# chintha/U-VIP-SLAM

Hardware: AMD Instinct MI355X
Metric: frames/sec ORB extract+match, 640x512 @1000 kp (higher is better)
Workload: dtype u8; 1 GPU; BASELINE.json configs[2]: 1xMI355X per rank, batch=256 synthetic 640x512 mono frames (+1 halo frame: the neighbouring rank's first), 1000 feats, 8 levels, fastTh 20, FullDetect extract + all-pairs 256-bit Hamming knn-2 of consecutive frames, HBM-resident I/O; batch_per_gpu=256, pipeline_depth=2, input_batches_in_rotation=4, fast_mode=adaptive

## Files before the change

u-vip-slam_amd/__init__.py:

```python
import ctypes
import os

import numpy as np

_HERE = os.path.dirname(os.path.abspath(__file__))
LIB_PATH = os.path.join(_HERE, "libuvo.so")

KEYPOINT_DTYPE = np.dtype([("x", "<f4"), ("y", "<f4"), ("size", "<f4"), ("angle", "<f4"), ("response", "<f4"), ("octave", "<i4"),
                           ("class_id", "<i4")])
assert KEYPOINT_DTYPE.itemsize == 28

UVO_OK, UVO_E_BADARG, UVO_E_NODEVICE, UVO_E_HIP, UVO_E_CAPACITY, UVO_E_UNSUPPORTED, UVO_E_NOMEM = 0, -1, -2, -3, -4, -5, -6
UVO_TUNE_OCT_WIDE_MAX = 1
UVO_TUNE_FAST_MODE = 2
UVO_FAST_MODE_ADAPTIVE, UVO_FAST_MODE_TWO_PASS, UVO_FAST_MODE_SINGLE_PASS = 0, 1, 2
UVO_TUNE_BLUR_ROUNDING, UVO_BLUR_ROUNDING_SCALAR, UVO_BLUR_ROUNDING_SSE2 = 9, 0, 1
UVO_TUNE_LEVEL0_INPLACE = 11
UVO_TUNE_FUSE_BLUR_TREE = 10
UVO_TUNE_PYR_RING = 12
UVO_TUNE_PYR_FORM, UVO_PYR_FORM_AUTO, UVO_PYR_FORM_LEVELS, UVO_PYR_FORM_TILES = 13, 0, 1, 2
UVO_TUNE_PYR_TILE_GROUP = 14
UVO_TUNE_FEW_FRAMES = 16
UVO_TUNE_ZERO_COPY_OUT, UVO_TUNE_SPIN_WAIT = 17, 18

ABI_SYMBOLS = [
    "uvo_extractor_create", "uvo_extractor_destroy", "uvo_extractor_levels", "uvo_extractor_max_keypoints", "uvo_extractor_scale_factor", "uvo_extractor_tables",
    "uvo_extract", "uvo_extract_tracked", "uvo_extract_batch", "uvo_extract_batch_device", "uvo_host_alloc", "uvo_host_free", "uvo_host_register", "uvo_host_unregister", "uvo_host_bind_near_device", "uvo_host_bind_to_cpulist_file", "uvo_shard_plan_make", "uvo_sharder_create", "uvo_sharder_destroy", "uvo_sharder_max_keypoints", "uvo_sharder_run", "uvo_sharder_submit", "uvo_sharder_wait", "uvo_extract_batch_submit", "uvo_extract_batch_wait", "uvo_extractor_synchronize", "uvo_extractor_set_pipeline", "uvo_extractor_tune", "uvo_extractor_fast_state", "uvo_extractor_level_dims",
    "uvo_grider_fast", "uvo_clahe", "uvo_clahe_batch_device", "uvo_extractor_read_plane", "uvo_extractor_read_candidates", "uvo_extractor_profile", "uvo_extractor_profile_only", "uvo_extractor_kernel_times",
    "uvo_matcher_create", "uvo_matcher_destroy", "uvo_matcher_synchronize", "uvo_hamming_knn2", "uvo_hamming_knn2_batch_device",
    "uvo_hamming_matrix", "uvo_distinctive_descriptors", "uvo_search_by_projection", "uvo_match_windows", "uvo_match_groups",
    "uvo_search_by_projection_kf", "uvo_search_by_bow", "uvo_search_for_triangulation", "uvo_search_for_triangulation_batch", "uvo_search_for_triangulation_next", "uvo_triangulate_matches", "uvo_create_new_map_points", "uvo_fuse", "uvo_fuse_batch", "uvo_project_points", "uvo_search_points_in_frustum", "uvo_sim3_decompose", "uvo_sim3_relative", "uvo_project_sim3", "uvo_search_by_projection_sim3", "uvo_search_by_sim3", "uvo_haloc_hash", "uvo_klt_create", "uvo_klt_destroy", "uvo_klt_build_pyramid", "uvo_klt_build_pyramid_from_extractor", "uvo_klt_read_level", "uvo_klt_track", "uvo_undistort_points", "uvo_klt_track_undistorted", "uvo_klt_find_fundamental", "uvo_klt_track_filtered", "uvo_klt_fm_hypotheses", "uvo_klt_solve_pnp_ransac", "uvo_klt_pnp_hypotheses", "uvo_vocabulary_create", "uvo_vocabulary_destroy", "uvo_bow_transform", "uvo_matcher_wait_extractor", "uvo_extractor_wait_matcher", "uvo_matcher_attach_extractor", "uvo_matcher_profile",
    "uvo_glibc_srand", "uvo_glibc_rand_next", "uvo_pnpsolver_set_create", "uvo_pnpsolver_set_destroy", "uvo_pnpsolver_set_clear", "uvo_pnpsolver_add",
    "uvo_pnpsolver_query", "uvo_pnpsolver_iterate", "uvo_pnpsolver_hypotheses",
    "uvo_sim3solver_set_create", "uvo_sim3solver_set_destroy", "uvo_sim3solver_set_clear", "uvo_sim3solver_add", "uvo_sim3solver_set_ransac_parameters",
    "uvo_sim3solver_query", "uvo_sim3solver_iterate", "uvo_sim3solver_find", "uvo_sim3solver_hypotheses",
    "uvo_initializer_create", "uvo_initializer_destroy", "uvo_initializer_set_reference", "uvo_initializer_initialize", "uvo_initializer_hypotheses",
    "uvo_matcher_kernel_times", "uvo_last_error", "uvo_device_info",
]


class MatchRule(ctypes.Structure):
    _fields_ = [("rule", ctypes.c_int32), ("max_dist", ctypes.c_int32), ("nn_ratio", ctypes.c_float), ("exclusive", ctypes.c_int32),
                ("check_orientation", ctypes.c_int32)]


class FeatureVectorC(ctypes.Structure):
    _fields_ = [("node", ctypes.c_void_p), ("start", ctypes.c_void_p), ("feat", ctypes.c_void_p), ("n_nodes", ctypes.c_int32)]


class Epipolar(ctypes.Structure):
    _fields_ = [("f12", ctypes.c_float * 9), ("q_x", ctypes.c_void_p), ("q_y", ctypes.c_void_p), ("t_x", ctypes.c_void_p), ("t_y", ctypes.c_void_p),
                ("sigma2", ctypes.c_void_p), ("nlevels", ctypes.c_int32)]


class CameraPose(ctypes.Structure):
    _fields_ = [("rcw", ctypes.c_float * 9), ("tcw", ctypes.c_float * 3), ("ow", ctypes.c_float * 3), ("fx", ctypes.c_float), ("fy", ctypes.c_float),
                ("cx", ctypes.c_float), ("cy", ctypes.c_float), ("min_x", ctypes.c_float), ("max_x", ctypes.c_float), ("min_y", ctypes.c_float),
                ("max_y", ctypes.c_float)]

    @classmethod
    def make(cls, Rcw, tcw, Ow, fx, fy, cx, cy, bounds):
        c = cls()
        c.rcw[:] = [float(x) for x in np.asarray(Rcw, np.float32).reshape(9)]
        c.tcw[:] = [float(x) for x in np.asarray(tcw, np.float32).reshape(3)]
        c.ow[:] = [float(x) for x in np.asarray(Ow, np.float32).reshape(3)]
        c.fx, c.fy, c.cx, c.cy = float(fx), float(fy), float(cx), float(cy)
        c.min_x, c.min_y, c.max_x, c.max_y = [float(b) for b in bounds]
        return c

    def as_array(self):
        return np.frombuffer(bytes(self), np.float32).copy()


# ... 1543 lines not shown
```

u-vip-slam_amd/csrc/common.hpp:

```cpp
#pragma once
#include "strip_plan.hpp"
#include "pyr_tiles.hpp"
#include <hip/hip_runtime.h>
#include <stdint.h>

#include "../../include/uvo/uvo.h"

namespace uvo {

constexpr int kMaxLevels = 16;
constexpr int kPad = 16;
constexpr int kPyrPitchAlign = 64;
constexpr int kMinBorder = 13;
constexpr int kMaxOctN = 2000;

struct LevelGeom {
  int w, h;
  int pw, ph, pitch;
  int64_t plane_off;
  int bw, bh;
  int nCols, nRows, wCell, hCell;
  int cell_base;
  int n_cells;
  int quota;
  int cand_cap;
  int64_t cand_off;
  int sel_cap;
  int sel_off;
  int nIni;
  float hX;
  float scale;
  float patch_size;
  int xtab_off;
  int ytab_off;
  int oct_tab_off;
  int pad_;
};

struct Level0View {
  const uint8_t* vbase;
  int64_t frame_stride;
  int pitch;
  int pad;
};

struct CellDesc {
  int16_t level;
  int16_t x0, y0;
  int16_t rw, rh;
  int16_t ox, oy;
  int16_t pad;
};

struct Geom {
  int width, height, nlevels;
  int total_cells;
  int64_t pyr_block;
  int64_t cand_block;
  int sel_block;
  int flist_cap;
  LevelGeom lv[kMaxLevels];
};


struct FinalSlot {
  float x, y;
  int32_t level;
  int32_t aux;
};

struct LaneScratch {
  uint8_t *pyr = nullptr, *blur = nullptr;
  uint32_t *cand_xy = nullptr, *cand_sc = nullptr, *cand_lo = nullptr, *pstate = nullptr, *sel_xy = nullptr, *sel_sc = nullptr;
  int32_t *cand_count = nullptr, *sel_count = nullptr, *n_final = nullptr, *cor_n = nullptr, *cursor = nullptr;
  uint32_t* cor = nullptr;
  uint8_t* cell_hi = nullptr;
  int32_t *tpass = nullptr, *fstat = nullptr, *fcount = nullptr;
  uint2* cell_list = nullptr;
  FinalSlot* flist = nullptr;
};

const char* hip_err_set(hipError_t e, const char* what);
#ifdef __HIPCC__
__device__ __forceinline__ int wave_in_block() { return __builtin_amdgcn_readfirstlane((int)(threadIdx.x >> 6)); }
#endif

int fail(int code, const char* msg);
int dev_malloc(void** p, size_t bytes);

#define UVO_HIP_CHECK(expr)                                   \
  do {                                                        \
    hipError_t _e = (expr);                                   \
    if (_e != hipSuccess) {                                   \
      uvo::hip_err_set(_e, #expr);                            \
      return UVO_E_HIP;                                       \
    }                                                         \
  } while (0)

#define RC(call)                   \
  do {                             \
    const int _rc = (call);        \
    if (_rc != UVO_OK) return _rc; \
  } while (0)

void launch_pad_level0(hipStream_t s, const uint8_t* d_img, int w, int h, int64_t stride, int64_t frame_stride, uint8_t* d_pyr,
                       int64_t pyr_block, const LevelGeom& g0, int batch);
void launch_resize_level(hipStream_t s, uint8_t* d_pyr, int64_t pyr_block, const LevelGeom& src, const LevelGeom& dst, const ResizeCol* d_ctab,
                         const ResizeRow* d_rtab, int fast_ok, int batch, Level0View l0, int ring);
constexpr int kPyrTilesMaxLds = 160 * 1024;
int prepare_pyr_tiles(uint32_t* max_lds);
int launch_pyr_tiles(hipStream_t s, uint8_t* d_pyr, int64_t pyr_block, const PyrTileLevel* d_plan, const Geom& g, const ResizeCol* d_ctab, const ResizeRow* d_rtab,
                     Level0View l0, int first, int last, int ntiles, uint32_t lds_bytes, int threads, int rows, int batch);
void launch_gauss7(hipStream_t s, const uint8_t* d_pyr, uint8_t* d_blur, int64_t pyr_block, const LevelGeom* d_lv, const Geom& g, int4 taps,
                   int batch, int sse2_rounding, Level0View l0);
void launch_fast_score(hipStream_t s, const LaneScratch& d, const Geom& g, int fast_th, int batch, Level0View l0);
void launch_fast_cells(hipStream_t s, const LaneScratch& d, const Geom& g, const CellDesc* d_cells, const int32_t* d_flag_cell, int batch, Level0View l0);
void launch_grider(hipStream_t s, const uint8_t* d_img, int w, int h, int64_t stride, int num_features, int grid_x, int grid_y, int threshold,
                   int nms, uint8_t* d_score, uint32_t* d_lists, int32_t* d_counts, uvo_keypoint* d_out, int cap, int32_t* d_n_out);
int fast_rows_per_seg(int batch);
int fast_items_per_frame(const Geom& g, int rows_per_seg);
int fast_flags_per_frame(const Geom& g);
struct OctLaunchState {
  int wide_max_problems = 0;
};
bool octree_gauss_applies(const OctLaunchState& st, const Geom& g, int batch);
void launch_octree_gauss(hipStream_t s, const LevelGeom* d_lv, const Geom& g, const LaneScratch& d, int4 taps, int sse2_rounding, int batch, Level0View l0,
                         const uint16_t* d_oct_tab);
int prepare_octree(const Geom& g);
void octree_fill_path_tables(const Geom& g, uint16_t* dst);
int launch_octree(hipStream_t s, OctLaunchState& st, const LevelGeom* d_lv, const Geom& g, const LaneScratch& d, int batch, const uint16_t* d_oct_tab);
struct FastAdapt {
  const int32_t* fcount;
  int32_t* tpass;
  int32_t* last;
  int adapt, fast_th;
};
void launch_assemble(hipStream_t s, const LevelGeom* d_lv, const Geom& g, FastAdapt fa, const LaneScratch& d, const int32_t* d_n_in, int in_cap,
                     int32_t* d_grid, int grid_rows, int grid_cols, int min_px_dist, int full_detect, const int32_t* d_nfn, int batch);
void launch_occupancy_grid(hipStream_t s, const uvo_keypoint* d_in_kp, const int32_t* d_n_in, int in_cap, int min_px_dist, int grid_rows, int grid_cols,
                           int32_t* d_grid, int batch);
void launch_knn2(hipStream_t s, int pairs, int max_q, const uint8_t* d_q, const int32_t* d_nq, int nq_fixed, int q_stride, const uint8_t* d_t,
                 const int32_t* d_nt, int nt_fixed, int t_stride, const uint8_t* d_mask, int out_stride, int32_t* d_idx0, uint16_t* d_d0,
                 int32_t* d_idx1, uint16_t* d_d1);
void launch_medoid(hipStream_t s, const uint8_t* d_desc, const int32_t* d_offsets, int npoints, int32_t* d_idx, int32_t* d_med);
void launch_matrix(hipStream_t s, const uint8_t* d_q, int nq, const uint8_t* d_t, int nt, uint16_t* d_dist);
void launch_grid_build(hipStream_t s, const uvo_keypoint* d_kp, const uint8_t* d_desc, int n, int min_x, int min_y, int max_x, int max_y,
                       int32_t* d_cell_start, int32_t* d_cell_items, int32_t* d_cell_of_kp);
void launch_sbp(hipStream_t s, const uvo_keypoint* d_kp, int n, const uint8_t* d_desc, int min_x, int min_y, int max_x, int max_y,
                int32_t* d_assigned, int nmp, const float* d_px, const float* d_py, const int32_t* d_level, const float* d_vc,
                const uint8_t* d_inview, const uint8_t* d_mpdesc, const float* d_scale, float th, float nnratio, int32_t* d_cell_start,
                int32_t* d_cell_items, int32_t* d_cell_of_kp, int32_t* d_cand_cnt, int32_t* d_cand_start, uint32_t* d_cand, int32_t* d_owner,
                int32_t* d_owner_next, int32_t* d_choice, int32_t* d_n_matches, int stage, int64_t cand_cap);
void launch_project(hipStream_t s, int mode, const uvo_camera_pose& cam, int n, const float* d_xyz, const float* d_normal, const float* d_min,
                    const float* d_max, const float* d_max_raw, const uint8_t* d_usable, const float* d_sf, int nlevels, float log_sf, float cos_limit,
                    uint8_t* d_valid, float* d_u, float* d_v, int32_t* d_level, float* d_cos);
void launch_project_sim3(hipStream_t s, const float* r_own, const float* t_own, const float* s_r, const float* t, const uvo_camera_pose& cam, int n,
                         const float* d_xyz, const float* d_min, const float* d_max, const uint8_t* d_usable, const float* d_sf, int nlevels,
                         uint8_t* d_valid, float* d_u, float* d_v, int32_t* d_level);
void launch_haloc(hipStream_t s, const float* d_proj, int num_proj, int proj_stride, const uint8_t* d_desc, int n, float* d_hash);
void launch_win_count(hipStream_t s, const uvo_keypoint* d_kp, const uint8_t* d_desc, int n, int min_x, int min_y, int max_x, int max_y, int nq,
                      const float* d_qx, const float* d_qy, const float* d_qr, const int32_t* d_qmin, const int32_t* d_qmax,
// ... 37 lines not shown
```

u-vip-slam_amd/csrc/extractor.cpp:

```cpp
#include <algorithm>
#include <chrono>
#include <cstdio>
#include <cstring>
#include <mutex>
#include <vector>

#include "extractor_priv.hpp"
#include "fast_geom.hpp"

namespace uvo {

static thread_local char g_err[512] = "";
const char* hip_err_set(hipError_t e, const char* what) {
  snprintf(g_err, sizeof(g_err), "HIP error %d (%s) in %s", (int)e, hipGetErrorString(e), what);
  return g_err;
}
int fail(int code, const char* msg) {
  snprintf(g_err, sizeof(g_err), "%s", msg);
  return code;
}

int dev_malloc(void** p, size_t bytes) {
  const hipError_t e = hipMalloc(p, bytes);
  if (e != hipSuccess) {
// ... 143 lines not shown

struct ProfScope : Profiler::Scope {
  ProfScope(uvo_extractor* h, const char* name) : Profiler::Scope(&h->prof, name, h->lane[h->cur].stream) {}
};

int run_batch_device(uvo_extractor* h, int li, const Batch& b) {
  if (!h || !b.imgs || !b.out_kp || !b.out_desc || !b.n_out) return fail(UVO_E_BADARG, "null pointer");
  const int batch = b.n, width = b.width, height = b.height, cap = b.cap, full_detect = b.full_detect;
  const ptrdiff_t stride = b.stride, frame_stride = b.frame_stride;
  const uint8_t* const d_imgs = b.imgs;
  if (batch < 1 || batch > h->cfg.max_batch) return fail(UVO_E_BADARG, "batch outside 1..max_batch");
  if (width < 1 || height < 1 || stride < width || cap < 1) return fail(UVO_E_BADARG, "bad image size / stride / cap");
  if (!full_detect && (!b.grid || !b.nfn || b.min_px_dist < 1 || b.grid_rows < 1 || b.grid_cols < 1))
    return fail(UVO_E_BADARG, "top-up mode needs grid2d, num_feats_needed and min_px_dist >= 1");
  if (!full_detect && (b.grid_rows <= (height - 1) / b.min_px_dist || b.grid_cols <= (width - 1) / b.min_px_dist))
    return fail(UVO_E_BADARG, "grid2d smaller than ceil(image / min_px_dist)");
  UVO_HIP_CHECK(hipSetDevice(h->device));
  int rc = set_geometry(h, width, height);
  if (rc) return rc;
  if ((rc = prepare_octree(h->geom)) != UVO_OK) return rc;
  h->cur = li;
  Lane& L = h->lane[li];
  hipStream_t s = L.stream;
  {
    std::lock_guard<std::mutex> lk(h->followers_mu);
    for (uvo_matcher* m : h->followers) uvo_matcher_follow_internal(m, s);
  }
  h->last_batch = batch;
  const Geom& g = h->geom;
  hipEvent_t& done = L.done[L.n_enqueued & 1];
  if (done) UVO_HIP_CHECK(hipEventSynchronize(done));
  else UVO_HIP_CHECK(hipEventCreateWithFlags(&done, hipEventDisableTiming));
  const bool have_in = b.in_kp && b.n_in;
  const bool inplace = h->level0_inplace && width % 4 == 0 && stride % 4 == 0 && frame_stride % 4 == 0 &&
                       (uintptr_t)d_imgs % 4 == 0 && !have_in && width >= 64 && height >= 64 &&
                       stride <= (1 << 20) && (int64_t)(height + 2 * kPad) * stride < (int64_t)1 << 31;
  Level0View l0{nullptr, 0, 0, 0};
  if (inplace) l0 = Level0View{d_imgs - (int64_t)kPad * stride - kPad, (int64_t)frame_stride, (int)stride, 0};
  L.l0_src = inplace ? d_imgs : nullptr, L.l0_stride = stride, L.l0_frame_stride = frame_stride;
  L.ring_used = h->pyr_ring;
  const Level0View no_l0{nullptr, 0, 0, 0};
  {
    if (!inplace) {
      ProfScope p(h, "k_pad_level0");
      launch_pad_level0(s, d_imgs, width, height, stride, frame_stride, L.d.pyr, g.pyr_block, g.lv[0], batch);
    }
    const bool tiles = h->pyr_ring == 4 && !h->tile_groups.empty() && (h->pyr_form == UVO_PYR_FORM_TILES || (h->pyr_form == UVO_PYR_FORM_AUTO && batch <= kTilePyramidFrames));
    if (tiles) {
      for (const TileGroup& G : h->tile_groups) {
        ProfScope p(h, "k_pyr_tiles");
        launch_pyr_tiles(s, L.d.pyr, g.pyr_block, G.d_plan, g, h->d_ctab, h->d_rtab, l0, G.first, G.last, G.tx * G.ty, G.lds, G.threads, G.rows, batch);
      }
    } else {
      for (int l = 1; l < g.nlevels; ++l) {
        ProfScope p(h, "k_resize_level");
        launch_resize_level(s, L.d.pyr, g.pyr_block, g.lv[l - 1], g.lv[l], h->d_ctab + g.lv[l].xtab_off, h->d_rtab + g.lv[l].ytab_off, h->resize_fast[l],
                            batch, l == 1 ? l0 : no_l0, h->pyr_ring);
      }
    }
  }
  const bool fused_tree = h->fuse_blur_tree && octree_gauss_applies(h->oct, g, batch);
  const bool few = batch <= kFewFrames && h->few_frames_shape;
  const int4 gtaps = make_int4(h->gtaps[0], h->gtaps[1], h->gtaps[2], h->gtaps[3]);
  {
    ProfScope p(h, "k_fast_score");
    launch_fast_score(s, L.d, g, h->cfg.fast_th, batch, l0);
  }
  if (h->cfg.fast_th > 7 && h->fast_mode != UVO_FAST_MODE_SINGLE_PASS) {
    ProfScope p(h, "k_fast_cells");
    launch_fast_cells(s, L.d, g, h->d_cells, h->d_cell_flag, batch, l0);
  }
  if (fused_tree) {
    ProfScope p(h, "k_octree_gauss");
    launch_octree_gauss(s, h->d_lv, g, L.d, gtaps, h->blur_rounding, batch, l0, h->d_oct_tab);
  } else {
    {
      ProfScope p(h, "k_gauss7");
      launch_gauss7(s, L.d.pyr, L.d.blur, g.pyr_block, h->d_lv, g, gtaps, batch, h->blur_rounding, l0);
    }
    {
      ProfScope p(h, "k_octree");
      rc = launch_octree(s, h->oct, h->d_lv, g, L.d, batch, h->d_oct_tab);
      if (rc) return rc;
    }
  }
  const bool direct = few && full_detect && !have_in;
  const FastAdapt fa{L.d.fcount, L.d.tpass, L.d.fstat, h->fast_mode == UVO_FAST_MODE_ADAPTIVE ? 1 : 0, h->cfg.fast_th};
  if (!direct) {
    ProfScope p(h, "k_assemble");
    launch_assemble(s, h->d_lv, g, fa, L.d, b.n_in, h->cfg.max_input_keypoints, b.grid, b.grid_rows, b.grid_cols, b.min_px_dist, full_detect, b.nfn, batch);
  }
  {
    ProfScope p(h, "k_describe");
    if (direct) launch_describe_direct(s, h->d_lv, g, L.d, fa, h->d_pattern, h->d_patch, b.out_kp, b.out_desc, cap, b.n_out, batch, l0);
    else launch_describe(s, h->d_lv, g, L.d, b.in_kp, h->cfg.max_input_keypoints, h->d_pattern, h->d_patch, b.out_kp, b.out_desc, cap, b.n_out, batch, l0);
  }
  UVO_HIP_CHECK(hipGetLastError());
  UVO_HIP_CHECK(hipEventRecord(done, s));
  L.n_enqueued++;
  return UVO_OK;
}

static int fill_lane(uvo_extractor* h, int li) {
  Lane& L = h->lane[li];
  LaneScratch& d = L.d;
  const size_t B = (size_t)h->cfg.max_batch;
  const hipError_t e = hipStreamCreateWithFlags(&L.stream, hipStreamNonBlocking);
  if (e != hipSuccess) {
    L.stream = nullptr;
    hip_err_set(e, "hipStreamCreate");
// ... 208 lines not shown
                           double clip_limit, int tiles_x, int tiles_y, uint8_t* d_dst, ptrdiff_t dst_stride, ptrdiff_t dst_frame_stride) {
  if (!h || !d_imgs || !d_dst) return fail(UVO_E_BADARG, "null pointer");
  if (stride < width || dst_stride < width) return fail(UVO_E_BADARG, "stride smaller than the row");
  UVO_HIP_CHECK(hipSetDevice(h->device));
  int tw, th, clip;
  float scale;
  int rc = clahe_setup(h, batch, width, height, clip_limit, tiles_x, tiles_y, &tw, &th, &clip, &scale);
  if (rc) return rc;
  Lane& L = h->lane[next_lane(h)];
  {
    Profiler::Scope ps(&h->prof, "k_clahe", L.stream);
    launch_clahe(L.stream, d_imgs, width, height, stride, frame_stride, batch, tiles_x, tiles_y, tw, th, clip, scale, h->d_clahe_lut, d_dst, dst_stride,
                 dst_frame_stride);
  }
  UVO_HIP_CHECK(hipGetLastError());
  return UVO_OK;
}

int uvo_extractor_max_keypoints(const uvo_extractor* h) {
  if (!h) return fail(UVO_E_BADARG, "null handle");
  return h->cap_flist;
}

int uvo_extractor_synchronize(uvo_extractor* h) {
  if (!h) return fail(UVO_E_BADARG, "null handle");
  UVO_HIP_CHECK(hipSetDevice(h->device));
  if (h->spin_wait && h->last_batch > 0 && h->last_batch <= 16) {
    for (int i = 0; i < kMaxLanes; ++i)
      if (h->lane[i].stream) UVO_HIP_CHECK(wait_stream(h->lane[i].stream, true));
    return UVO_OK;
  }
  return sync_all_lanes(h);
}

int uvo_extractor_tune(uvo_extractor* h, int knob, int value) {
  if (!h) return fail(UVO_E_BADARG, "null handle");
  switch (knob) {
    case UVO_TUNE_OCT_WIDE_MAX:
      if (value < 0) return fail(UVO_E_BADARG, "knob value must be >= 0");
      h->oct.wide_max_problems = value;
      return UVO_OK;
    case UVO_TUNE_FAST_MODE: {
      if (value != UVO_FAST_MODE_ADAPTIVE && value != UVO_FAST_MODE_TWO_PASS && value != UVO_FAST_MODE_SINGLE_PASS)
        return fail(UVO_E_BADARG, "UVO_TUNE_FAST_MODE takes UVO_FAST_MODE_ADAPTIVE / _TWO_PASS / _SINGLE_PASS");
      UVO_HIP_CHECK(hipSetDevice(h->device));
      int rc = sync_all_lanes(h);
      if (rc) return rc;
      h->fast_mode = value;
      for (int i = 0; i < kMaxLanes; ++i)
        if (h->lane[i].stream && (rc = set_lane_fast_mode(h, i)) != UVO_OK) return rc;
      return UVO_OK;
    }
    case UVO_TUNE_PYR_FORM:
      if (value < UVO_PYR_FORM_AUTO || value > UVO_PYR_FORM_TILES) return fail(UVO_E_BADARG, "UVO_TUNE_PYR_FORM takes UVO_PYR_FORM_AUTO / _LEVELS / _TILES");
      h->pyr_form = value;
      return UVO_OK;
    case UVO_TUNE_PYR_TILE_GROUP: {
      const int first = (value >> 16) & 0xff, tx = (value >> 8) & 0xff, ty = value & 0xff;
      if (value != 0 && (first < 1 || first >= kMaxLevels || tx < 1 || ty < 1 || (first > 1 && (h->tile_spec.empty() || first <= (int)((h->tile_spec.back() >> 16) & 0xff)))))
        return fail(UVO_E_BADARG, "UVO_TUNE_PYR_TILE_GROUP takes first << 16 | tx << 8 | ty with ascending first levels starting at 1, or 0");
      UVO_HIP_CHECK(hipSetDevice(h->device));
      int rc = sync_all_lanes(h);
      if (rc) return rc;
      if (value == 0 || first == 1) h->tile_spec.clear();
      if (value != 0) h->tile_spec.push_back((uint32_t)value);
      return h->have_geom ? build_tile_groups(h, h->geom) : UVO_OK;
    }
    case UVO_TUNE_PYR_RING:
      if (value != 0 && value != 4 && value != 8 && value != 12) return fail(UVO_E_BADARG, "UVO_TUNE_PYR_RING takes 0, 4, 8 or 12");
      h->pyr_ring = value;
      return UVO_OK;
    case UVO_TUNE_LEVEL0_INPLACE:
      h->level0_inplace = value != 0;
      return UVO_OK;
    case UVO_TUNE_ZERO_COPY_OUT:
      h->zero_copy_out = value != 0;
      return UVO_OK;
    case UVO_TUNE_SPIN_WAIT:
      h->spin_wait = value != 0;
      return UVO_OK;
    case UVO_TUNE_FEW_FRAMES:
      h->few_frames_shape = value != 0;
      return UVO_OK;
    case UVO_TUNE_FUSE_BLUR_TREE:
      h->fuse_blur_tree = value != 0;
      return UVO_OK;
    case UVO_TUNE_BLUR_ROUNDING:
      if (value != UVO_BLUR_ROUNDING_SCALAR && value != UVO_BLUR_ROUNDING_SSE2) return fail(UVO_E_BADARG, "UVO_TUNE_BLUR_ROUNDING takes UVO_BLUR_ROUNDING_SCALAR / _SSE2");
      h->blur_rounding = value;
      return UVO_OK;
    default:
      return fail(UVO_E_BADARG, "unknown knob");
  }
}

int uvo_extractor_fast_state(uvo_extractor* h, int32_t* pass_threshold, int32_t* fallback_cells, int32_t* cells_per_frame) {
  if (!h) return fail(UVO_E_BADARG, "null handle");
  if (!h->have_geom) return fail(UVO_E_BADARG, "no batch has run yet");
  UVO_HIP_CHECK(hipSetDevice(h->device));
  Lane& L = h->lane[h->cur];
  UVO_HIP_CHECK(hipStreamSynchronize(L.stream));
  int32_t t[kMaxLevels], f[kMaxLevels];
  UVO_HIP_CHECK(hipMemcpy(t, L.d.tpass, sizeof(t), hipMemcpyDeviceToHost));
  UVO_HIP_CHECK(hipMemcpy(f, L.d.fstat, sizeof(f), hipMemcpyDeviceToHost));
  for (int l = 0; l < h->geom.nlevels; ++l) {
    if (pass_threshold) pass_threshold[l] = t[l];
    if (fallback_cells) fallback_cells[l] = f[l];
// ... 124 lines not shown
```

u-vip-slam_amd/csrc/pyramid.hip:

```cpp
#include "common.hpp"
#include <algorithm>
#include <cstring>
#include <mutex>

namespace uvo {

__device__ __forceinline__ int reflect101(int p, int len) {
  p = p < 0 ? -p : p;
  p = p >= len ? 2 * (len - 1) - p : p;
  return p;
}

__global__ __launch_bounds__(256) void k_pad_level0(const uint8_t* __restrict__ img, int w, int h, int64_t stride, int64_t frame_stride,
                                                    uint8_t* __restrict__ pyr, int64_t pyr_block, int64_t plane_off, int pitch, int ph,
                                                    int vec_ok) {
  const int qx = blockIdx.x * 64 + (threadIdx.x & 63);
  const int py = blockIdx.y * 4 + wave_in_block();
  const int f = blockIdx.z;
  if (qx * 16 >= pitch || py >= ph) return;
  const int y = reflect101(py - kPad, h);
  const uint8_t* src = img + f * frame_stride + (int64_t)y * stride;
  const int x0 = qx * 16 - kPad;
  uint4 v;
  const int r0 = x0 + 16 <= 0 ? -(x0 + 15) : 2 * (w - 1) - x0 - 15;
// ... 125 lines not shown
        L1 |= (uint32_t)S1[sx[i]] << (8 * i), R1 |= (uint32_t)S1[sx1] << (8 * i);
      }
    }
    const uint32_t b0s = (uint32_t)rr[j].b0 << 8, b1s = (uint32_t)rr[j].b1 << 8;
    uint32_t v = vrow(hrow<0>(L0, R0, a0[0], a1[0]), hrow<0>(L1, R1, a0[0], a1[0]), b0s, b1s);
    v |= vrow(hrow<1>(L0, R0, a0[1], a1[1]), hrow<1>(L1, R1, a0[1], a1[1]), b0s, b1s) << 8;
    v |= vrow(hrow<2>(L0, R0, a0[2], a1[2]), hrow<2>(L1, R1, a0[2], a1[2]), b0s, b1s) << 16;
    v |= vrow(hrow<3>(L0, R0, a0[3], a1[3]), hrow<3>(L1, R1, a0[3], a1[3]), b0s, b1s) << 24;
    vout[j] = v;
  }
  uint8_t* dst = pyr + f * pyr_block + dst_off + (int64_t)py0 * dst_pitch + wx * 4;
  if (py0 + RZ_ROWS <= dst_ph) {
#pragma unroll
    for (int j = 0; j < RZ_ROWS; ++j) *reinterpret_cast<uint32_t*>(dst + (uint32_t)(j * dst_pitch)) = vout[j];
  } else {
#pragma unroll
    for (int j = 0; j < RZ_ROWS; ++j)
      if (py0 + j < dst_ph) *reinterpret_cast<uint32_t*>(dst + (uint32_t)(j * dst_pitch)) = vout[j];
  }
}

void launch_pad_level0(hipStream_t s, const uint8_t* d_img, int w, int h, int64_t stride, int64_t frame_stride, uint8_t* d_pyr,
                       int64_t pyr_block, const LevelGeom& g0, int batch) {
  dim3 block(256);
  dim3 grid((g0.pitch / 16 + 63) / 64, (g0.ph + 3) / 4, batch);
  const int vec_ok = ((uintptr_t)d_img % 16 == 0 && stride % 16 == 0 && frame_stride % 16 == 0) ? 1 : 0;
  hipLaunchKernelGGL(k_pad_level0, grid, block, 0, s, d_img, w, h, stride, frame_stride, d_pyr, pyr_block, g0.plane_off, g0.pitch, g0.ph,
                     vec_ok);
}

void launch_resize_level(hipStream_t s, uint8_t* d_pyr, int64_t pyr_block, const LevelGeom& src, const LevelGeom& dst, const ResizeCol* d_ctab,
                         const ResizeRow* d_rtab, int fast_ok, int batch, Level0View l0, int ring) {
  dim3 block(256);
  uint32_t nwx = (uint32_t)dst.pitch / 4, groups = ((uint32_t)dst.ph + RZ_ROWS - 1) / RZ_ROWS;
  int wx0 = 0, rg0 = 0, row_end = dst.ph;
  if (ring > 0 && ring < kPad && (kPad - ring) % 4 == 0) {
    wx0 = (kPad - ring) / 4, rg0 = (kPad - ring) / RZ_ROWS, row_end = dst.h + kPad + ring;
    nwx = (uint32_t)((dst.w + kPad + ring + 3) / 4 - wx0), groups = (uint32_t)((row_end + RZ_ROWS - 1) / RZ_ROWS - rg0);
  }
  const uint32_t magic = (uint32_t)((0x100000000ull + nwx - 1) / nwx);
  const uint32_t per_frame = (nwx * groups + 255) / 256;
  const uint32_t pf_magic = (uint32_t)((0x100000000ull + per_frame - 1) / per_frame);
  const uint32_t max_frames = (uint32_t)std::min<uint64_t>(1u << 20, std::max<uint64_t>(1, 0xffffffffull / ((uint64_t)per_frame * per_frame)));
  for (int f0 = 0; f0 < batch; f0 += (int)max_frames) {
    const int nb = std::min<int>(batch - f0, (int)max_frames);
    const uint32_t per_xcd = (per_frame * (uint32_t)nb + 7) / 8;
    Level0View v = l0;
    if (v.vbase) v.vbase += (int64_t)f0 * v.frame_stride;
    hipLaunchKernelGGL(k_resize_level, dim3(8 * per_xcd), block, 0, s, d_pyr + (int64_t)f0 * pyr_block, pyr_block, src.plane_off, src.pitch, src.w, dst.plane_off, dst.pitch,
                       dst.ph, dst.w, fast_ok, d_ctab, d_rtab, magic, v, src.h, per_frame, pf_magic, per_xcd, nb, nwx, wx0, rg0, row_end);
  }
}


struct PyrTilesArgs {
  uint8_t* pyr;
  int64_t pyr_block;
  const PyrTileLevel* plan;
  const ResizeCol* ctab;
  const ResizeRow* rtab;
  Level0View l0;
  int nlevels, first, last, ntiles, batch;
  uint32_t ntiles_magic, per_xcd;
  int64_t src_plane_off;
  int src_pitch, src_w, src_h;
  int64_t plane_off[kMaxLevels];
  int pitch[kMaxLevels], xtab_off[kMaxLevels], ytab_off[kMaxLevels];
};

constexpr int kPyrTilesMaxGroup = 8;

template <bool FROM_LDS, int ROWS>
__device__ __forceinline__ void pyr_tile_level(const PyrTilesArgs& A, const PyrTileLevel& T, const PyrTileLevel& SP, int l, int f, uint8_t* lds) {
  static_assert(ROWS == 1 || ROWS == RZ_ROWS, "items are single rows or row groups of the row table");
  const ResizeCol* __restrict__ ct = A.ctab + A.xtab_off[l];
  const ResizeRow* __restrict__ rt = A.rtab + A.ytab_off[l];
  const uint4* __restrict__ tabs = reinterpret_cast<const uint4*>(lds + T.tab_off);
  const int ncw = (int)T.ncw;
  const int nitems = ncw * (int)T.nrg * (RZ_ROWS / ROWS);
  const bool ip = !FROM_LDS && l == 1 && A.l0.vbase != nullptr;
  const int src_pitch = FROM_LDS ? (int)SP.lw + kPyrTileSlack : (ip ? A.l0.pitch : A.src_pitch);
  const uint8_t* S = nullptr;
  if (!FROM_LDS) S = ip ? A.l0.vbase + f * A.l0.frame_stride + (int64_t)kPad * src_pitch + kPad : A.pyr + f * A.pyr_block + A.src_plane_off + (int64_t)kPad * src_pitch + kPad;
  const uint8_t* SLDS = lds + SP.lds_off - ((int)SP.ly0 * src_pitch + (int)SP.lx0);
  const int sw = A.src_w, sh = A.src_h;
  const int64_t s_end = ip ? (int64_t)(sh - 1) * src_pitch + sw : INT64_MAX;
  uint8_t* dplane = A.pyr + f * A.pyr_block + A.plane_off[l];
  const int dpitch = A.pitch[l];
  const int tpitch = (int)T.lw + kPyrTileSlack;
  uint8_t* TL = lds + T.lds_off;
  for (int it = (int)threadIdx.x; it < nitems; it += (int)blockDim.x) {
    const int rl = (int)__umulhi((uint32_t)it, T.ncw_magic);
    const int cwl = it - rl * ncw;
    const int wx = (int)T.cx0w + cwl;
    const int py0 = (int)T.cy0 + rl * ROWS;
    uint4 c01, c23;
    uint32_t tw[2 * ROWS];
    if (FROM_LDS) {
      c01 = tabs[2 * cwl], c23 = tabs[2 * cwl + 1];
      if (ROWS == RZ_ROWS) {
        const uint4 t01 = tabs[2 * ncw + 2 * rl], t23 = tabs[2 * ncw + 2 * rl + 1];
        const uint32_t q[8] = {t01.x, t01.y, t01.z, t01.w, t23.x, t23.y, t23.z, t23.w};
#pragma unroll
        for (int j = 0; j < 2 * ROWS; ++j) tw[j] = q[j];
      } else {
        const uint2 t0 = reinterpret_cast<const uint2*>(tabs + 2 * ncw)[rl];
// ... 176 lines not shown
```

u-vip-slam_amd/csrc/tune_internal.h:

```cpp
#pragma once
#define UVO_TUNE_PYR_RING 12
#define UVO_TUNE_FUSE_BLUR_TREE 10
#define UVO_TUNE_PYR_FORM 13
#define UVO_PYR_FORM_AUTO 0
#define UVO_PYR_FORM_LEVELS 1
#define UVO_PYR_FORM_TILES 2
#define UVO_TUNE_PYR_TILE_GROUP 14
#define UVO_TUNE_FEW_FRAMES 16
#define UVO_TUNE_ZERO_COPY_OUT 17
#define UVO_TUNE_SPIN_WAIT 18
```

Before: 312,900 frames/s.

## Add row-band resize kernel reusing horizontally filtered source rows across outputs

Adds a new pyramid resize kernel in which each wavefront walks a vertical band of 16 output rows. It broadcasts the row tables through readlane, prefetches source rows a few steps ahead, and caches horizontally filtered rows so a source row shared by consecutive outputs is filtered only once. This is meant to cut the redundant loads and horizontal filtering of the per-row resize kernel. AUTO mode now selects it when the batch exceeds the tile-pyramid threshold and there is enough work. The cost is more code paths, guard handling for level-0 views, and serial per-band work that may reduce parallelism.

```diff
diff --git a/u-vip-slam_amd/__init__.py b/u-vip-slam_amd/__init__.py
--- a/u-vip-slam_amd/__init__.py
+++ b/u-vip-slam_amd/__init__.py
@@ -18,7 +18,7 @@
 UVO_TUNE_LEVEL0_INPLACE = 11
 UVO_TUNE_FUSE_BLUR_TREE = 10
 UVO_TUNE_PYR_RING = 12
-UVO_TUNE_PYR_FORM, UVO_PYR_FORM_AUTO, UVO_PYR_FORM_LEVELS, UVO_PYR_FORM_TILES = 13, 0, 1, 2
+UVO_TUNE_PYR_FORM, UVO_PYR_FORM_AUTO, UVO_PYR_FORM_LEVELS, UVO_PYR_FORM_TILES, UVO_PYR_FORM_ROWS = 13, 0, 1, 2, 3
 UVO_TUNE_PYR_TILE_GROUP = 14
 UVO_TUNE_FEW_FRAMES = 16
 UVO_TUNE_ZERO_COPY_OUT, UVO_TUNE_SPIN_WAIT = 17, 18
diff --git a/u-vip-slam_amd/csrc/common.hpp b/u-vip-slam_amd/csrc/common.hpp
--- a/u-vip-slam_amd/csrc/common.hpp
+++ b/u-vip-slam_amd/csrc/common.hpp
@@ -1,6 +1,7 @@
 #pragma once
 #include "strip_plan.hpp"
 #include "pyr_tiles.hpp"
+#include "resize_rows.hpp"
 #include <hip/hip_runtime.h>
 #include <stdint.h>
 
@@ -107,6 +108,9 @@
                        int64_t pyr_block, const LevelGeom& g0, int batch);
 void launch_resize_level(hipStream_t s, uint8_t* d_pyr, int64_t pyr_block, const LevelGeom& src, const LevelGeom& dst, const ResizeCol* d_ctab,
                          const ResizeRow* d_rtab, int fast_ok, int batch, Level0View l0, int ring);
+bool resize_level_rows_applies(const LevelGeom& src, const LevelGeom& dst, int fast_ok, int batch, Level0View l0, int ring, int64_t pyr_block, bool forced);
+void launch_resize_level_rows(hipStream_t s, uint8_t* d_pyr, int64_t pyr_block, const LevelGeom& src, const LevelGeom& dst, const ResizeCol* d_ctab,
+                              const ResizeRow* d_rtab, int batch, Level0View l0, int ring);
 constexpr int kPyrTilesMaxLds = 160 * 1024;
 int prepare_pyr_tiles(uint32_t* max_lds);
 int launch_pyr_tiles(hipStream_t s, uint8_t* d_pyr, int64_t pyr_block, const PyrTileLevel* d_plan, const Geom& g, const ResizeCol* d_ctab, const ResizeRow* d_rtab,
diff --git a/u-vip-slam_amd/csrc/extractor.cpp b/u-vip-slam_amd/csrc/extractor.cpp
--- a/u-vip-slam_amd/csrc/extractor.cpp
+++ b/u-vip-slam_amd/csrc/extractor.cpp
@@ -219,10 +219,18 @@
         launch_pyr_tiles(s, L.d.pyr, g.pyr_block, G.d_plan, g, h->d_ctab, h->d_rtab, l0, G.first, G.last, G.tx * G.ty, G.lds, G.threads, G.rows, batch);
       }
     } else {
+      const bool rows = h->pyr_form == UVO_PYR_FORM_ROWS || (h->pyr_form == UVO_PYR_FORM_AUTO && batch > kTilePyramidFrames);
       for (int l = 1; l < g.nlevels; ++l) {
-        ProfScope p(h, "k_resize_level");
-        launch_resize_level(s, L.d.pyr, g.pyr_block, g.lv[l - 1], g.lv[l], h->d_ctab + g.lv[l].xtab_off, h->d_rtab + g.lv[l].ytab_off, h->resize_fast[l],
-                            batch, l == 1 ? l0 : no_l0, h->pyr_ring);
+        const Level0View v = l == 1 ? l0 : no_l0;
+        const ResizeCol* ct = h->d_ctab + g.lv[l].xtab_off;
+        const ResizeRow* rt = h->d_rtab + g.lv[l].ytab_off;
+        if (rows && resize_level_rows_applies(g.lv[l - 1], g.lv[l], h->resize_fast[l], batch, v, h->pyr_ring, g.pyr_block, h->pyr_form == UVO_PYR_FORM_ROWS)) {
+          ProfScope p(h, "k_resize_level_rows");
+          launch_resize_level_rows(s, L.d.pyr, g.pyr_block, g.lv[l - 1], g.lv[l], ct, rt, batch, v, h->pyr_ring);
+        } else {
+          ProfScope p(h, "k_resize_level");
+          launch_resize_level(s, L.d.pyr, g.pyr_block, g.lv[l - 1], g.lv[l], ct, rt, h->resize_fast[l], batch, v, h->pyr_ring);
+        }
       }
     }
   }
@@ -537,7 +545,7 @@
       return UVO_OK;
     }
     case UVO_TUNE_PYR_FORM:
-      if (value < UVO_PYR_FORM_AUTO || value > UVO_PYR_FORM_TILES) return fail(UVO_E_BADARG, "UVO_TUNE_PYR_FORM takes UVO_PYR_FORM_AUTO / _LEVELS / _TILES");
+      if (value < UVO_PYR_FORM_AUTO || value > UVO_PYR_FORM_ROWS) return fail(UVO_E_BADARG, "UVO_TUNE_PYR_FORM takes UVO_PYR_FORM_AUTO / _LEVELS / _TILES / _ROWS");
       h->pyr_form = value;
       return UVO_OK;
     case UVO_TUNE_PYR_TILE_GROUP: {
diff --git a/u-vip-slam_amd/csrc/pyramid.hip b/u-vip-slam_amd/csrc/pyramid.hip
--- a/u-vip-slam_amd/csrc/pyramid.hip
+++ b/u-vip-slam_amd/csrc/pyramid.hip
@@ -201,6 +201,165 @@
   }
 }
 
+struct ResizeRowsArgs {
+  const uint8_t* src;
+  uint8_t* dst;
+  uint32_t src_frame, dst_frame;
+  int src_pitch, dst_pitch, sh;
+  int guard;
+  uint32_t guard_lim;
+  const ResizeCol* ctab;
+  const ResizeRow* rtab;
+  int rtab_last;
+  ResizeRowsRegion r;
+  uint32_t nwx_magic, nbands_magic, entries, nitems, per_xcd;
+};
+
+static_assert(UVO_RESIZE_AHEAD >= 1 && UVO_RESIZE_BAND >= 2 && UVO_RESIZE_BAND + UVO_RESIZE_AHEAD <= 64,
+              "lane j of a wavefront holds the table entry of the band's row j, lanes n .. n + UVO_RESIZE_AHEAD - 1 the look-ahead's");
+
+template <bool GUARD>
+__device__ __forceinline__ void rows_load(const uint8_t* __restrict__ S, int sy, int pitch, uint32_t vsrc, uint32_t glim, uint32_t (&u)[3]) {
+  const uint32_t ro = (uint32_t)sy * (uint32_t)pitch;
+  if (!GUARD) {
+    const uint8_t* p = S + ro;
+#pragma unroll
+    for (int k = 0; k < 3; ++k) u[k] = *reinterpret_cast<const uint32_t*>(p + (uint64_t)vsrc + 4 * k);
+  } else {
+#pragma unroll
+    for (int k = 0; k < 3; ++k) u[k] = *reinterpret_cast<const uint32_t*>(S + (uint64_t)(vsrc + min(ro + 4u * k, glim)));
+  }
+}
+__device__ __forceinline__ void rows_hfilter(const uint32_t (&u)[3], uint32_t sel, const uint32_t (&a0)[4], const uint32_t (&a1)[4], uint32_t (&q)[4]) {
+  const uint32_t L = __builtin_amdgcn_perm(u[1], u[0], sel);
+  const uint32_t R = __builtin_amdgcn_perm(__builtin_amdgcn_alignbyte(u[2], u[1], 1), __builtin_amdgcn_alignbyte(u[1], u[0], 1), sel);
+  q[0] = hrow<0>(L, R, a0[0], a1[0]), q[1] = hrow<1>(L, R, a0[1], a1[1]), q[2] = hrow<2>(L, R, a0[2], a1[2]), q[3] = hrow<3>(L, R, a0[3], a1[3]);
+}
+__device__ __forceinline__ uint32_t rows_vfilter(const uint32_t (&q0)[4], const uint32_t (&q1)[4], uint32_t b0s, uint32_t b1s) {
+  return vrow(q0[0], q1[0], b0s, b1s) | vrow(q0[1], q1[1], b0s, b1s) << 8 | vrow(q0[2], q1[2], b0s, b1s) << 16 | vrow(q0[3], q1[3], b0s, b1s) << 24;
+}
+
+struct RowsLane {
+  uint32_t a0[4], a1[4], sel;
+  uint32_t vsrc, glim, vdst;
+  uint32_t tsy, tb;
+};
+
+template <bool GUARD>
+__device__ __forceinline__ void rows_walk(const ResizeRowsArgs& A, const RowsLane& T, int py0, int n) {
+  constexpr int AH = UVO_RESIZE_AHEAD, R = AH + 1, U = R % 2 ? 2 * R : R;
+  const uint8_t* __restrict__ S = A.src;
+  uint8_t* drow = A.dst + (int64_t)py0 * A.dst_pitch;
+  const int spitch = A.src_pitch;
+  uint32_t slot[2][4] = {{0, 0, 0, 0}, {0, 0, 0, 0}};
+  ResizeRowsState st{{-1, -1}};
+  uint32_t ua[R][3], ub[R][3];
+  ResizeRowsStep stp[R];
+#pragma unroll
+  for (int k = 0; k < AH; ++k) {
+    const uint32_t e = (uint32_t)__builtin_amdgcn_readlane((int)T.tsy, k);
+    stp[k] = resize_rows_step(st, k & 1, (int)(e & 0xffffu), (int)(e >> 16));
+    if (stp[k].eval0) rows_load<GUARD>(S, (int)(e & 0xffffu), spitch, T.vsrc, T.glim, ua[k]);
+    rows_load<GUARD>(S, (int)(e >> 16), spitch, T.vsrc, T.glim, ub[k]);
+  }
+  for (int j = 0;; j += U) {
+#pragma unroll
+    for (int k = 0; k < U; ++k) {
+      const int c = k % R, nx = (k + AH) % R, p = k & 1;
+      const uint32_t e = (uint32_t)__builtin_amdgcn_readlane((int)T.tsy, j + k + AH);
+      stp[nx] = resize_rows_step(st, (k + AH) & 1, (int)(e & 0xffffu), (int)(e >> 16));
+      if (stp[nx].eval0) rows_load<GUARD>(S, (int)(e & 0xffffu), spitch, T.vsrc, T.glim, ua[nx]);
+      rows_load<GUARD>(S, (int)(e >> 16), spitch, T.vsrc, T.glim, ub[nx]);
+      const uint32_t bw = (uint32_t)__builtin_amdgcn_readlane((int)T.tb, j + k);
+      const uint32_t b0s = (bw & 0xffffu) << 8, b1s = (bw >> 16) << 8;
+      if (stp[c].eval0) rows_hfilter(ua[c], T.sel, T.a0, T.a1, slot[p]);
+      rows_hfilter(ub[c], T.sel, T.a0, T.a1, slot[p ^ 1]);
+      *reinterpret_cast<uint32_t*>(drow + (uint64_t)T.vdst) = rows_vfilter(slot[p], slot[p ^ 1], b0s, b1s);
+      drow += A.dst_pitch;
+      if (j + k + 1 >= n) return;
+    }
+  }
+}
+
+#ifndef UVO_OCC_RESIZE_ROWS
+#define UVO_OCC_RESIZE_ROWS 8
+#endif
+__global__ __launch_bounds__(256, UVO_OCC_RESIZE_ROWS) void k_resize_level_rows(ResizeRowsArgs A) {
+  const uint32_t vb = (blockIdx.x & 7u) * A.per_xcd + (blockIdx.x >> 3);
+  const uint32_t item = vb * 4u + (uint32_t)wave_in_block();
+  if (item >= A.nitems) return;
+  const uint32_t chunk = __umulhi(item, A.nbands_magic);
+  const int band = (int)(item - chunk * (uint32_t)A.r.nbands);
+  int py0, n;
+  resize_rows_band(A.r, band, &py0, &n);
+  const uint32_t lane = threadIdx.x & 63u;
+  RowsLane T;
+  const uint32_t ent = chunk * 64u + lane;
+  const uint32_t en = min(ent, A.entries - 1u);
+  const uint32_t f = __umulhi(en, A.nwx_magic);
+  const int wx = (int)(en - f * (uint32_t)A.r.nwx) + A.r.wx0;
+  const uint4 c01 = reinterpret_cast<const uint4*>(A.ctab)[wx * 2], c23 = reinterpret_cast<const uint4*>(A.ctab)[wx * 2 + 1];
+  const uint32_t cw[8] = {c01.x, c01.y, c01.z, c01.w, c23.x, c23.y, c23.z, c23.w};
+#pragma unroll
+  for (int i = 0; i < 4; ++i) T.a0[i] = cw[2 * i] >> 16, T.a1[i] = cw[2 * i + 1] & 0xffffu;
+  const uint32_t base = cw[1] >> 16;
+  T.sel = (cw[3] >> 16) | (cw[5] & 0xffff0000u);
+  T.vsrc = f * A.src_frame + base;
+  T.vdst = f * A.dst_frame + (uint32_t)wx * 4u;
+  T.glim = A.guard_lim - base;
+  const uint2 te = reinterpret_cast<const uint2*>(A.rtab)[min(py0 + (int)lane, A.rtab_last)];
+  T.tsy = te.x, T.tb = te.y;
+  const bool guard = A.guard && __ballot((int)lane < n + UVO_RESIZE_AHEAD && (int)(te.x >> 16) >= A.sh - 1) != 0ull;
+  if (guard) rows_walk<true>(A, T, py0, n);
+  else rows_walk<false>(A, T, py0, n);
+}
+
+#ifndef UVO_RESIZE_ROWS_MIN_ITEMS
+#define UVO_RESIZE_ROWS_MIN_ITEMS 2048
+#endif
+
+static int64_t resize_rows_frames(const LevelGeom& src, const LevelGeom& dst, int fast_ok, Level0View l0, int ring, int64_t pyr_block) {
+  if (!fast_ok) return 0;
+  const ResizeRowsRegion r = resize_rows_region(dst.w, dst.h, dst.pitch, ring);
+  int64_t frame_bytes = pyr_block;
+  if (l0.vbase) {
+    if (l0.frame_stride < (int64_t)(src.h - 1) * l0.pitch + src.w) return 0;
+    frame_bytes = std::max<int64_t>(frame_bytes, l0.frame_stride);
+  }
+  return resize_rows_max_frames(r.nwx, r.nbands, frame_bytes);
+}
+
+bool resize_level_rows_applies(const LevelGeom& src, const LevelGeom& dst, int fast_ok, int batch, Level0View l0, int ring, int64_t pyr_block, bool forced) {
+  if (resize_rows_frames(src, dst, fast_ok, l0, ring, pyr_block) < 1) return false;
+  if (forced) return true;
+  const ResizeRowsRegion r = resize_rows_region(dst.w, dst.h, dst.pitch, ring);
+  return ((int64_t)batch * r.nwx + 63) / 64 * r.nbands >= UVO_RESIZE_ROWS_MIN_ITEMS;
+}
+
+void launch_resize_level_rows(hipStream_t s, uint8_t* d_pyr, int64_t pyr_block, const LevelGeom& src, const LevelGeom& dst, const ResizeCol* d_ctab,
+                              const ResizeRow* d_rtab, int batch, Level0View l0, int ring) {
+  const int max_frames = (int)resize_rows_frames(src, dst, 1, l0, ring, pyr_block);
+  ResizeRowsArgs A;
+  memset(&A, 0, sizeof(A));
+  A.r = resize_rows_region(dst.w, dst.h, dst.pitch, ring);
+  A.src_pitch = l0.vbase ? l0.pitch : src.pitch, A.dst_pitch = dst.pitch, A.sh = src.h;
+  A.src_frame = (uint32_t)(l0.vbase ? l0.frame_stride : pyr_block), A.dst_frame = (uint32_t)pyr_block;
+  A.guard = l0.vbase != nullptr;
+  A.guard_lim = (uint32_t)((int64_t)(src.h - 1) * A.src_pitch + src.w - 4);
+  A.ctab = d_ctab, A.rtab = d_rtab, A.rtab_last = ((dst.ph + 3) & ~3) - 1;
+  A.nwx_magic = (uint32_t)((0x100000000ull + (uint32_t)A.r.nwx - 1) / (uint32_t)A.r.nwx);
+  A.nbands_magic = (uint32_t)((0x100000000ull + (uint32_t)A.r.nbands - 1) / (uint32_t)A.r.nbands);
+  for (int f0 = 0; f0 < batch; f0 += max_frames) {
+    const int nb = std::min(batch - f0, max_frames);
+    A.src = l0.vbase ? l0.vbase + (int64_t)f0 * l0.frame_stride + (int64_t)kPad * l0.pitch + kPad
+                     : d_pyr + (int64_t)f0 * pyr_block + src.plane_off + (int64_t)kPad * src.pitch + kPad;
+    A.dst = d_pyr + (int64_t)f0 * pyr_block + dst.plane_off;
+    A.entries = (uint32_t)nb * (uint32_t)A.r.nwx;
+    A.nitems = (A.entries + 63u) / 64u * (uint32_t)A.r.nbands;
+    A.per_xcd = ((A.nitems + 3u) / 4u + 7u) / 8u;
+    hipLaunchKernelGGL(k_resize_level_rows, dim3(8 * A.per_xcd), dim3(256), 0, s, A);
+  }
+}
 
 struct PyrTilesArgs {
   uint8_t* pyr;
diff --git a/u-vip-slam_amd/csrc/resize_rows.hpp b/u-vip-slam_amd/csrc/resize_rows.hpp
--- /dev/null
+++ b/u-vip-slam_amd/csrc/resize_rows.hpp
@@ -0,0 +1,64 @@
+#pragma once
+#include <stdint.h>
+
+#ifndef UVO_RESIZE_BAND
+#define UVO_RESIZE_BAND 16
+#endif
+#ifndef UVO_RESIZE_AHEAD
+#define UVO_RESIZE_AHEAD 3
+#endif
+
+#if defined(__HIPCC__)
+#define UVO_RR_HD __host__ __device__ inline __attribute__((always_inline))
+#else
+#define UVO_RR_HD inline
+#endif
+
+namespace uvo {
+
+constexpr int kResizeRowsPad = 16;
+
+struct ResizeRowsRegion {
+  int wx0, nwx, row0, row_end, nbands;
+};
+UVO_RR_HD ResizeRowsRegion resize_rows_region(int dw, int dh, int dpitch, int ring) {
+  ResizeRowsRegion r;
+  r.wx0 = 0, r.nwx = dpitch / 4, r.row0 = 0, r.row_end = dh + 2 * kResizeRowsPad;
+  if (ring > 0 && ring < kResizeRowsPad && (kResizeRowsPad - ring) % 4 == 0) {
+    r.wx0 = (kResizeRowsPad - ring) / 4, r.row0 = kResizeRowsPad - ring, r.row_end = dh + kResizeRowsPad + ring;
+    r.nwx = (dw + kResizeRowsPad + ring + 3) / 4 - r.wx0;
+  }
+  r.nbands = (r.row_end - r.row0 + UVO_RESIZE_BAND - 1) / UVO_RESIZE_BAND;
+  return r;
+}
+UVO_RR_HD void resize_rows_band(const ResizeRowsRegion& r, int b, int* py0, int* n) {
+  *py0 = r.row0 + b * UVO_RESIZE_BAND;
+  const int left = r.row_end - *py0;
+  *n = left < UVO_RESIZE_BAND ? left : UVO_RESIZE_BAND;
+}
+
+struct ResizeRowsState {
+  int tag[2];
+};
+struct ResizeRowsStep {
+  int eval0, eval1;
+};
+UVO_RR_HD ResizeRowsStep resize_rows_step(ResizeRowsState& st, int p, int sy0, int sy1) {
+  ResizeRowsStep s;
+  s.eval0 = (p ? st.tag[1] : st.tag[0]) != sy0;
+  s.eval1 = (p ? st.tag[0] : st.tag[1]) != sy1;
+  st.tag[0] = p ? sy1 : sy0, st.tag[1] = p ? sy0 : sy1;
+  return s;
+}
+
+inline int64_t resize_rows_max_frames(int nwx, int nbands, int64_t frame_bytes) {
+  if (frame_bytes <= 0 || nwx <= 0 || nbands <= 0) return 0;
+  const int64_t a = 0xffffffffll / ((int64_t)nwx * nwx), b = 0xffffffffll / frame_bytes;
+  const int64_t c = (0xffffffffll / ((int64_t)nbands * nbands) - 1) * 64 / nwx;
+  int64_t m = a < b ? a : b;
+  m = c < m ? c : m;
+  m = m < 0 ? 0 : m;
+  return m < (1 << 20) ? m : (1 << 20);
+}
+
+}
diff --git a/u-vip-slam_amd/csrc/tune_internal.h b/u-vip-slam_amd/csrc/tune_internal.h
--- a/u-vip-slam_amd/csrc/tune_internal.h
+++ b/u-vip-slam_amd/csrc/tune_internal.h
@@ -5,6 +5,7 @@
 #define UVO_PYR_FORM_AUTO 0
 #define UVO_PYR_FORM_LEVELS 1
 #define UVO_PYR_FORM_TILES 2
+#define UVO_PYR_FORM_ROWS 3
 #define UVO_TUNE_PYR_TILE_GROUP 14
 #define UVO_TUNE_FEW_FRAMES 16
 #define UVO_TUNE_ZERO_COPY_OUT 17
```

Result: faster. 321,200 frames/s (median of 6 runs) (+2.6%).
